# Chriz122/ultralytics_pro

Measured on AMD Instinct MI355X. Metric: images/sec (whole job = n_gpus x per-GPU bs=32) YOLOv8n 640x640 (forward + Detect decode + NMS), higher is better.
Workload: dtype bf16

## Files before the change

include/upa.h:

```cpp
#ifndef UPA_H
#define UPA_H
#include <stddef.h>
#include <stdint.h>

#ifdef __cplusplus
extern "C" {
#endif

enum { UPA_F32 = 0, UPA_BF16 = 1, UPA_U8_BGR_HWC = 2  };
enum { UPA_ACT_NONE = 0, UPA_ACT_SILU = 1, UPA_ACT_RELU = 2 };
enum { UPA_OK = 0, UPA_EINVAL = -1, UPA_EUNSUPPORTED = -2, UPA_EWORKSPACE = -3, UPA_ELAUNCH = -4 };

typedef struct upa_opts {
  uint32_t size;
  int32_t conv_big;
  int32_t conv_big_bm;
  int32_t conv_ckt;
  int32_t no_ws, no_pipe, no_1x1, no_c16, no_upcat;
  int32_t pipe_all;
  int32_t pipe_min_tiles;
  int32_t pipe_wgs, c16_wgs;
  int32_t c1_mt, c1_waves, c1_wgs;
  int32_t pair;
  int32_t pair_tile64, pair_tile32;
  int32_t no_pair_cv2;
  int32_t c2f;
  int32_t c2f16_waves;
  int32_t c2f32_th;
  int32_t no_branch_tail;
  int32_t branch_tail_bm;
  int32_t stem_wgs, stemf_wgs, stemf_waves, stem_no_mfma;
  int32_t ablate_conv, ablate_pipe, ablate_c1, ablate_stem;
  int32_t c2f64_max_px;
  int32_t conv_ws3;
  int32_t no_group;
  int32_t no_c2f32_up;
  int32_t no_xcd;
  int32_t keys_only;
  int32_t conv_p8;
  int32_t c2f_stream;
  int32_t c2f_stream_rows;
  int32_t no_stack_first;
  int32_t no_epi_stats;
  int32_t nms_stages;
  int32_t nms_first_prefix;
  int32_t detect_stream;
  int32_t detect_stream_rows;
  int32_t no_sppf_front;
  int32_t no_c2f16_down;
} upa_opts;

int upa_version(void);
const char* upa_last_error(void);
size_t upa_opts_size(void);

size_t upa_conv_packed_weight_bytes(int cout, int cin, int k, int dtype);
int upa_pack_conv_weight(const float* w_oihw, int cout, int cin, int k, int dtype, void* out);
int upa_conv2d_bias_act(const void* x, int n, int h, int w, int cin, int ldx,
                        const void* w_packed, const float* bias ,
                        void* y, int cout, int ldy,
                        const void* residual , int ldr,
                        int k, int stride, int pad, int act, int dtype, const upa_opts* opts, void* stream);
typedef struct upa_conv_problem {
  const void* x; int32_t n, h, w, cin, ldx;
  const void* w_packed; const float* bias;
  void* y; int32_t cout, ldy;
  const void* residual; int32_t ldr;
} upa_conv_problem;
int upa_conv2d_bias_act_group(const upa_conv_problem* probs, int count, int k, int stride, int pad, int act, int dtype,
                              const upa_opts* opts, void* stream);

int upa_conv2d_pool2(const void* x, int n, int h, int w, int cin, int ldx, const void* w_packed, const float* bias, void* y, int cout,
                     int ldy, int k, int stride, int pad, int act, int dtype, const upa_opts* opts, void* stream);
int upa_conv2d_stem_nchw_pool2(const void* x_nchw, int x_dtype, int n, int cin, int h, int w, const float* w_oihw, const float* bias,
                               void* y, int cout, int ldy, int k, int stride, int pad, int act, int dtype, const upa_opts* opts,
                               void* stream);

int upa_conv_variant(int n, int h, int w, int cin, int cout, int k, int stride, int pad, int dtype, const upa_opts* opts);

int upa_bottleneck_pair(const void* x, int n, int h, int w, int c, int ldx, const void* w1_packed, const float* b1,
                        const void* w2_packed, const float* b2, void* y, int ldy, int residual, int act, int dtype,
                        const upa_opts* opts, void* stream);
int upa_bottleneck_pair_e(const void* x, int n, int h, int w, int c, int cmid, int ldx, const void* w1_packed, const float* b1,
                          const void* w2_packed, const float* b2, void* y, int ldy, int residual, int act, int dtype,
                          const upa_opts* opts, void* stream);


size_t upa_stem_packed_weight_bytes(int cout, int cin, int k);
int upa_pack_stem_weight(const float* w_oihw, int cout, int cin, int k, float* out );
int upa_conv2d_stem_nchw(const void* x_nchw, int x_dtype, int n, int cin, int h, int w,
                         const float* w_oihw, const float* bias, void* y, int cout, int ldy,
                         int k, int stride, int pad, int act, int dtype, const upa_opts* opts, void* stream);

enum { UPA_STEM_SCALAR = 1, UPA_STEM_MFMA = 2, UPA_STEM_MFMA_G16 = 3, UPA_STEM_FUSED16 = 4, UPA_STEM_FUSED32 = 5 };
enum { UPA_STEM_STAGE_DMA = 0, UPA_STEM_STAGE_VGPR = 1, UPA_STEM_STAGE_U8 = 2 };
long long upa_stem_variant(int x_dtype, int n, int cin, int h, int w, int cout, int ldy, int k, int stride, int pad, int act, int dtype,
                           int pool, const upa_opts* opts, int x_align);

int upa_stem_conv_fused(const void* x, int n, int h, int w, const float* w0, const float* b0, const void* w1,
                        const float* b1, void* y, int ldy, const upa_opts* opts, void* stream);
int upa_stem_conv_fused_k(const void* x, int n, int h, int w, int k0, const float* w0, const float* b0, const void* w1,
                          const float* b1, void* y, int ldy, const upa_opts* opts, void* stream);
int upa_stem_conv_fused_c(const void* x, int n, int h, int w, int k0, int c0, const float* w0, const float* b0, const void* w1,
                          const float* b1, void* y, int ldy, const upa_opts* opts, void* stream);
int upa_stem_conv_fused_s(const void* x, int n, int h, int w, int k0, int s0, int c0, const float* w0, const float* b0,
                          const void* w1, const float* b1, void* y, int ldy, const upa_opts* opts, void* stream);

long long upa_stem_fused_variant(int n, int h, int w, int k0, int s0, int c0, int ldy, const upa_opts* opts, int x_align);

int upa_maxpool2d(const void* x, int n, int h, int w, int c, int ldx, void* y, int oh, int ow, int ldy,
                  int k, int stride, int pad, int pad_br, int dtype, void* stream);
int upa_sppf_pool3(const void* x, int n, int h, int w, int c, int ldx, void* y1, void* y2, void* y3, int ldy,
                   int dtype, void* stream);
int upa_sppf_front(const void* x, int n, int h, int w, int c1, int ldx, const void* w_packed, const float* bias, void* y, int c_, int ldy, int dtype,
                   const upa_opts* opts, void* stream);
int upa_upsample2x(const void* x, int n, int h, int w, int c, int ldx, void* y, int ldy, int dtype, void* stream);
int upa_copy_view(const void* x, int n, int h, int w, int c, int ldx, void* y, int ldy, int dtype, void* stream);
int upa_copy_to_host(const void* src_dev, void* dst_pinned, size_t bytes, void* stream);
int upa_results_to_host(const void* rows_dev, const int* counts_dev, int batch, int max_rows, int row_bytes,
                        void* rows_pinned, int* counts_pinned, void* stream);
int upa_add_view(const void* a, int lda, const void* b, int ldb, void* y, int ldy, int n, int h, int w, int c,
                 int dtype, void* stream);
int upa_nchw_to_nhwc(const float* x, int n, int c, int h, int w, void* y, int ldy, int dtype, void* stream);
int upa_nhwc_to_nchw(const void* x, int n, int h, int w, int c, int ldx, float* y, int dtype, void* stream);
int upa_letterbox_u8(const void* src, int n, int h0, int w0, long src_image_stride, int src_row_stride, void* dst, int H, int W,
                     int new_h, int new_w, int top, int left, int pad_value, void* stream);


int upa_detect_decode(const void* box, int ldb, const void* cls, int ldc, int n, int h, int w, int reg_max, int nc,
                      float stride_px, float* y, int a_total, int a0, int dtype, void* stream);
int upa_detect_tail(const void* x, int n, int h, int w, int cin, int ldx, const void* w_packed, const float* bias, int cout,
                    int kind, int nc, float stride_px, float* y, int a_total, int a0, void* raw, int ldraw,
// ... 284 lines not shown
```

ultralytics_pro_amd/_lib.py:

```python

from __future__ import annotations

import ctypes as C
import os
from pathlib import Path

import torch

UPA_F32, UPA_BF16, UPA_U8_BGR_HWC = 0, 1, 2
UPA_EINVAL = -1
UPA_EUNSUPPORTED = -2
ACT_NONE, ACT_SILU, ACT_RELU = 0, 1, 2
MASKS_PLANES, MASKS_OVERLAP = 0, 1
MASK_U8, MASK_F32, MASK_I32 = 0, 1, 2

_PKG = Path(__file__).resolve().parent
LIB_PATH = Path(os.environ.get("UPA_HIP_LIB", _PKG / "libupa_hip.so"))

_vp, _i, _f, _sz = C.c_void_p, C.c_int, C.c_float, C.c_size_t


class Opts(C.Structure):

    _fields_ = [("size", C.c_uint32), ("conv_big", _i), ("conv_big_bm", _i), ("conv_ckt", _i),
                ("no_ws", _i), ("no_pipe", _i), ("no_1x1", _i), ("no_c16", _i), ("no_upcat", _i),
                ("pipe_all", _i), ("pipe_min_tiles", _i), ("pipe_wgs", _i), ("c16_wgs", _i),
                ("c1_mt", _i), ("c1_waves", _i), ("c1_wgs", _i),
                ("pair", _i), ("pair_tile64", _i), ("pair_tile32", _i), ("no_pair_cv2", _i),
                ("c2f", _i), ("c2f16_waves", _i), ("c2f32_th", _i),
                ("no_branch_tail", _i), ("branch_tail_bm", _i),
                ("stem_wgs", _i), ("stemf_wgs", _i), ("stemf_waves", _i), ("stem_no_mfma", _i),
                ("ablate_conv", _i), ("ablate_pipe", _i), ("ablate_c1", _i), ("ablate_stem", _i), ("c2f64_max_px", _i), ("conv_ws3", _i), ("no_group", _i), ("no_c2f32_up", _i), ("no_xcd", _i), ("keys_only", _i), ("conv_p8", _i), ("c2f_stream", _i), ("c2f_stream_rows", _i), ("no_stack_first", _i), ("no_epi_stats", _i), ("nms_stages", _i), ("nms_first_prefix", _i), ("detect_stream", _i), ("detect_stream_rows", _i), ("no_sppf_front", _i), ("no_c2f16_down", _i)]

    def __init__(self, **kw):
        super().__init__()
        self.size = C.sizeof(Opts)
        for k, v in kw.items():
            if k in dict(self._fields_):
                setattr(self, k, int(v))
            else:
                raise AttributeError(f"upa_opts has no field '{k}'")

    def replace(self, **kw) -> "Opts":
        o = Opts()
        C.memmove(C.byref(o), C.byref(self), C.sizeof(Opts))
        for k, v in kw.items():
            setattr(o, k, int(v))
        return o

    _ENV = {"UPA_CONV_BIG": ("conv_big", lambda v: {0: 1, 1: 0, 2: 2}[int(v)]), "UPA_CONV_BIG_BM": ("conv_big_bm", int), "UPA_CONV_WS3": ("conv_ws3", int),
            "UPA_CONV_CKT": ("conv_ckt", int), "UPA_CONV_NO_WS": ("no_ws", lambda v: 1), "UPA_CONV_NO_PIPE": ("no_pipe", lambda v: 1),
            "UPA_CONV_NO_1X1": ("no_1x1", lambda v: 1), "UPA_CONV_NO_C16": ("no_c16", lambda v: 1), "UPA_NO_UPCAT": ("no_upcat", lambda v: 1),
            "UPA_PIPE_ALL": ("pipe_all", lambda v: 1), "UPA_PIPE_MIN_TILES": ("pipe_min_tiles", int), "UPA_PIPE_WGS": ("pipe_wgs", int),
            "UPA_C16_WGS": ("c16_wgs", int), "UPA_C1_MT": ("c1_mt", int), "UPA_C1_WAVES": ("c1_waves", int), "UPA_C1_WGS": ("c1_wgs", int),
            "UPA_NO_PAIR": ("pair", lambda v: {0: 2, 1: 1, 2: 0, 3: 3}[int(v)]), "UPA_PAIR_T64": ("pair_tile64", int),
            "UPA_PAIR_T32": ("pair_tile32", int), "UPA_NO_PAIR_CV2": ("no_pair_cv2", int), "UPA_NO_C2F": ("c2f", int),
            "UPA_C2F16_WAVES": ("c2f16_waves", int), "UPA_C2F32_TH": ("c2f32_th", int), "UPA_NO_BRANCH_TAIL": ("no_branch_tail", int),
            "UPA_BRANCH_TAIL_BM": ("branch_tail_bm", int), "UPA_STEM_WGS": ("stem_wgs", int), "UPA_STEMF_WGS": ("stemf_wgs", int),
            "UPA_STEMF_WAVES": ("stemf_waves", int), "UPA_STEM_NO_MFMA": ("stem_no_mfma", lambda v: 1),
            "UPA_CONV_ABLATE": ("ablate_conv", int), "UPA_PIPE_ABLATE": ("ablate_pipe", int), "UPA_C1_ABLATE": ("ablate_c1", int),
            "UPA_STEM_ABLATE": ("ablate_stem", int)}

    @classmethod
    def from_env(cls, env=None) -> "Opts":
        env = os.environ if env is None else env
        o = cls()
        for name, (field, conv) in cls._ENV.items():
            if name in env:
                setattr(o, field, conv(env[name]))
        return o


class BranchLevel(C.Structure):
    _fields_ = [("x", C.c_void_p), ("n", _i), ("h", _i), ("w", _i), ("c", _i), ("ldx", _i), ("w3_packed", C.c_void_p), ("b3", C.c_void_p),
                ("wt_packed", C.c_void_p), ("bt", C.c_void_p), ("stride_px", C.c_float), ("a0", _i)]


class DetectBranch(C.Structure):
    _fields_ = [("c", _i), ("reserved", _i), ("w1", C.c_void_p), ("b1", C.c_void_p), ("w2", C.c_void_p), ("b2", C.c_void_p),
                ("wt", C.c_void_p), ("bt", C.c_void_p)]


class ConvProblem(C.Structure):
    _fields_ = [("x", C.c_void_p), ("n", _i), ("h", _i), ("w", _i), ("cin", _i), ("ldx", _i), ("w_packed", C.c_void_p), ("bias", C.c_void_p),
                ("y", C.c_void_p), ("cout", _i), ("ldy", _i), ("residual", C.c_void_p), ("ldr", _i)]


_op = C.POINTER(Opts)

PROTOTYPES = {
    "upa_version": (_i, []),
    "upa_last_error": (C.c_char_p, []),
    "upa_opts_size": (_sz, []),
    "upa_conv_packed_weight_bytes": (_sz, [_i, _i, _i, _i]),
    "upa_pack_conv_weight": (_i, [_vp, _i, _i, _i, _i, _vp]),
    "upa_conv2d_bias_act": (_i, [_vp, _i, _i, _i, _i, _i, _vp, _vp, _vp, _i, _i, _vp, _i, _i, _i, _i, _i, _i, _op, _vp]),
    "upa_conv_variant": (_i, [_i, _i, _i, _i, _i, _i, _i, _i, _i, _op]),
    "upa_bottleneck_pair": (_i, [_vp, _i, _i, _i, _i, _i, _vp, _vp, _vp, _vp, _vp, _i, _i, _i, _i, _op, _vp]),
    "upa_bottleneck_pair_e": (_i, [_vp, _i, _i, _i, _i, _i, _i, _vp, _vp, _vp, _vp, _vp, _i, _i, _i, _i, _op, _vp]),
    "upa_stem_packed_weight_bytes": (_sz, [_i, _i, _i]),
    "upa_pack_stem_weight": (_i, [_vp, _i, _i, _i, _vp]),
    "upa_conv2d_stem_nchw": (_i, [_vp, _i, _i, _i, _i, _i, _vp, _vp, _vp, _i, _i, _i, _i, _i, _i, _i, _op, _vp]),
    "upa_conv2d_stem_nchw_pool2": (_i, [_vp, _i, _i, _i, _i, _i, _vp, _vp, _vp, _i, _i, _i, _i, _i, _i, _i, _op, _vp]),
    "upa_conv2d_pool2": (_i, [_vp, _i, _i, _i, _i, _i, _vp, _vp, _vp, _i, _i, _i, _i, _i, _i, _i, _op, _vp]),
    "upa_stem_conv_fused": (_i, [_vp, _i, _i, _i, _vp, _vp, _vp, _vp, _vp, _i, _op, _vp]),
    "upa_stem_conv_fused_k": (_i, [_vp, _i, _i, _i, _i, _vp, _vp, _vp, _vp, _vp, _i, _op, _vp]),
    "upa_stem_conv_fused_c": (_i, [_vp, _i, _i, _i, _i, _i, _vp, _vp, _vp, _vp, _vp, _i, _op, _vp]),
    "upa_stem_conv_fused_s": (_i, [_vp, _i, _i, _i, _i, _i, _i, _vp, _vp, _vp, _vp, _vp, _i, _op, _vp]),
    "upa_stem_variant": (C.c_longlong, [_i, _i, _i, _i, _i, _i, _i, _i, _i, _i, _i, _i, _i, _op, _i]),
    "upa_stem_fused_variant": (C.c_longlong, [_i, _i, _i, _i, _i, _i, _i, _op, _i]),
    "upa_maxpool2d": (_i, [_vp, _i, _i, _i, _i, _i, _vp, _i, _i, _i, _i, _i, _i, _i, _i, _vp]),
    "upa_sppf_pool3": (_i, [_vp, _i, _i, _i, _i, _i, _vp, _vp, _vp, _i, _i, _vp]),
    "upa_upsample2x": (_i, [_vp, _i, _i, _i, _i, _i, _vp, _i, _i, _vp]),
    "upa_copy_view": (_i, [_vp, _i, _i, _i, _i, _i, _vp, _i, _i, _vp]),
    "upa_copy_to_host": (_i, [_vp, _vp, _sz, _vp]),
# ... 181 lines not shown
```

ultralytics_pro_amd/csrc/conv_big.hip:

```cpp
#include <stdlib.h>

#include <mutex>
#include <type_traits>
#include <unordered_map>

#include "common.h"
#include "conv_pipe.h"
UPA_STAMP_DEFINE(conv_big)

template <int KS, int STRIDE, int WM, int WN, int MT, int NT, int TAIL = 0>
__device__ __forceinline__ void conv_big_body(const BigParams& p, const int bid0) {
  static_assert(WM * WN == 8, "8 waves per workgroup");
  static_assert(TAIL == 0 || TAIL == 3 || TAIL == 4 || WN == 1, "a tail needs every channel of a pixel in one wave");
  static_assert(TAIL != 1 || (NT % 2) == 0, "box branch: 64 channels");
  static_assert(TAIL != 3 || (NT % 2) == 0, "the statistics epilogue pairs n-tiles");
  static_assert(TAIL != 4 || ((NT % 2) == 0 && KS == 2 && STRIDE == 1), "the interleaving epilogue: 2 x 2 phase kernels, paired n-tiles");
  constexpr int NTB = WN * NT;
  constexpr int WBUF = 2 * NTB * 1024;
  extern __shared__ __attribute__((aligned(16))) char smem[];
  const int tid = threadIdx.x;
  const int lane = tid & 63;
  const int wave = __builtin_amdgcn_readfirstlane(tid >> 6);
  const int r = lane & 15, g = lane >> 4;
  const int wm = wave / WN, wn = wave % WN;

  const int tilesPerImg = p.tilesX * p.tilesY;
  int bid = p.no_xcd ? bid0 : upa_xcd_tile(bid0, tilesPerImg * p.N);
  const int n = bid / tilesPerImg;
  bid -= n * tilesPerImg;
  const int tyi = bid / p.tilesX;
  const int txi = bid - tyi * p.tilesX;
  const int oy0 = tyi * p.TH, ox0 = txi * p.TW;
  const int iy0 = oy0 * STRIDE - p.pad, ix0 = ox0 * STRIDE - p.pad;
  const int ntb0 = blockIdx.y * NTB;

  const int haloItems = p.IH * p.IWp * 8;
  const int haloPadded = (haloItems + 63) & ~63;
  char* hal = smem;
  char* wbuf = smem + (size_t)haloPadded * 16;

  int pl0[MT], pty[MT], ptx[MT];
#pragma unroll
  for (int i = 0; i < MT; ++i) {
    const int pp = (wm * MT + i) * 16 + r;
    int ty = (int)__umulhi((unsigned)pp, p.magicTW);
    int tx = pp - ty * p.TW;
    if (ty >= p.TH) { ty = p.TH; tx = 0; }
    pty[i] = ty;
    ptx[i] = tx;
    pl0[i] = ty < p.TH ? (ty * STRIDE) * p.IWp + tx : 0;
  }

  f32x4 acc[MT][NT];
#pragma unroll
  for (int i = 0; i < MT; ++i)
#pragma unroll
    for (int j = 0; j < NT; ++j) acc[i][j] = f32x4{0.f, 0.f, 0.f, 0.f};

  constexpr int TAPS = KS * KS;
  const int nChunks = (p.KTT + 1) >> 1;

  auto stage_halo = [&](int c) __attribute__((always_inline)) {
    const int c0 = c * 64;
    for (int base = wave * 64; base < haloPadded; base += 512) {
      const int idx = base + lane;
      const int pix = idx >> 3;
      const int slot = idx & 7;
      const int cg = slot ^ (pix & 7);
      const int py = (int)__umulhi((unsigned)pix, p.magicIW);
      const int qx = pix - py * p.IWp;
      int px = qx;
      if constexpr (STRIDE == 2) px = qx < p.HALF ? 2 * qx : 2 * (qx - p.HALF) + 1;
      const int iy = iy0 + py, ix = ix0 + px;
      const int ch = c0 + cg * 8;
      const char* src = reinterpret_cast<const char*>(g_zero16);
      if (idx < haloItems && px < p.IW && iy >= 0 && iy < p.H && ix >= 0 && ix < p.W && ch < p.Cin)
        src = p.x + ((((size_t)n * p.H + iy) * p.W + ix) * (size_t)p.ldx + ch) * 2;
      lds_dma16(src, hal + base * 16);
    }
  };
  auto stage_w = [&](int c, int tap, int b) __attribute__((always_inline)) {
#pragma unroll
    for (int f0 = 0; f0 < 2 * NTB; f0 += 8) {
      const int f = f0 + wave;
      if (f < 2 * NTB) {
        const int kt = f / NTB, j = f - kt * NTB;
        const int ktg = c * 2 + kt;
        const int nt = ntb0 + j;
        const char* src = reinterpret_cast<const char*>(g_zero16);
        if (ktg < p.KTT && nt < p.NTn) src = p.w + (((size_t)(tap * p.KTT + ktg) * p.NTn + nt) * 64 + lane) * 16;
        lds_dma16(src, wbuf + b * WBUF + f * 1024);
      }
    }
  };

  UPA_STAMP_AT(0);
  UPA_STAMP_HWID();
  stage_halo(0);
  stage_w(0, 0, 0);
  int buf = 0;
  for (int c = 0; c < nChunks; ++c) {
    int kh = 0, kw = 0;
#pragma unroll 1
    for (int tap = 0; tap < TAPS; ++tap) {
      asm volatile("s_waitcnt vmcnt(0)" ::: "memory");
      __syncthreads();
      if (c == 0) UPA_STAMP_AT(1 + tap);
      if (tap + 1 < TAPS) stage_w(c, tap + 1, buf ^ 1);
      const int tapshift = kh * p.IWp + (STRIDE == 2 ? (kw >> 1) + (kw & 1) * p.HALF : kw);
      const char* wb = wbuf + buf * WBUF + (wn * NT) * 1024 + lane * 16;
      int paddr[MT], pswz[MT];
#pragma unroll
      for (int i = 0; i < MT; ++i) {
        const int pl = pl0[i] + tapshift;
        paddr[i] = pl * 128;
        pswz[i] = pl & 7;
      }
#pragma unroll
      for (int kt = 0; kt < 2; ++kt) {
        if constexpr (TAIL == 2) {
          if (kt == 1 && c * 2 + 1 >= p.KTT) break;
        }
        if constexpr (NT <= 6) {
          u32x4 a[NT], b[MT];
#pragma unroll
          for (int j = 0; j < NT; ++j) a[j] = *reinterpret_cast<const u32x4*>(wb + (kt * NTB + j) * 1024);
#pragma unroll
          for (int i = 0; i < MT; ++i) b[i] = *reinterpret_cast<const u32x4*>(hal + paddr[i] + (((kt * 4 + g) ^ pswz[i]) << 4));
#pragma unroll
          for (int i = 0; i < MT; ++i)
#pragma unroll
            for (int j = 0; j < NT; ++j)
              acc[i][j] = __builtin_amdgcn_mfma_f32_16x16x32_bf16(*reinterpret_cast<const bf16x8*>(&a[j]),
                                                                  *reinterpret_cast<const bf16x8*>(&b[i]), acc[i][j], 0, 0, 0);
        } else {
          constexpr int GS = (NT + 1) / 2;
          u32x4 b[MT];
#pragma unroll
          for (int i = 0; i < MT; ++i) b[i] = *reinterpret_cast<const u32x4*>(hal + paddr[i] + (((kt * 4 + g) ^ pswz[i]) << 4));
#pragma unroll
          for (int j0 = 0; j0 < NT; j0 += GS) {
            u32x4 a[GS];
#pragma unroll
            for (int j = 0; j < GS; ++j)
              if (j0 + j < NT) a[j] = *reinterpret_cast<const u32x4*>(wb + (kt * NTB + j0 + j) * 1024);
#pragma unroll
            for (int i = 0; i < MT; ++i)
#pragma unroll
              for (int j = 0; j < GS; ++j)
                if (j0 + j < NT)
                  acc[i][j0 + j] = __builtin_amdgcn_mfma_f32_16x16x32_bf16(*reinterpret_cast<const bf16x8*>(&a[j]),
                                                                           *reinterpret_cast<const bf16x8*>(&b[i]), acc[i][j0 + j], 0, 0, 0);
            __builtin_amdgcn_sched_barrier(0);
          }
        }
      }
      buf ^= 1;
      if (++kw == KS) { kw = 0; ++kh; }
    }
    if (c + 1 < nChunks) {
      __syncthreads();
      stage_halo(c + 1);
      stage_w(c + 1, 0, buf);
    }
  }
  UPA_STAMP_AT(10);

  if constexpr (TAIL == 1 || TAIL == 2) {
    f32x4 bv[NT];
#pragma unroll
    for (int j = 0; j < NT; ++j) bv[j] = *reinterpret_cast<const f32x4*>(p.bias + j * 16 + g * 4);
    f32x4 acc2[MT][NT];
#pragma unroll
    for (int i = 0; i < MT; ++i)
#pragma unroll
      for (int j = 0; j < NT; ++j) acc2[i][j] = f32x4{0.f, 0.f, 0.f, 0.f};
#pragma unroll
    for (int s2 = 0; s2 < NT / 2; ++s2) {
      u32x4 hb[MT];
#pragma unroll
      for (int i = 0; i < MT; ++i) {
        float v0[4], v1[4];
#pragma unroll
        for (int q = 0; q < 4; ++q) {
          v0[q] = act_rcp<UPA_ACT_SILU>(acc[i][2 * s2][q] + bv[2 * s2][q]);
          v1[q] = act_rcp<UPA_ACT_SILU>(acc[i][2 * s2 + 1][q] + bv[2 * s2 + 1][q]);
        }
        hb[i] = u32x4{pack_bf16x2(v0[0], v0[1]), pack_bf16x2(v0[2], v0[3]), pack_bf16x2(v1[0], v1[1]), pack_bf16x2(v1[2], v1[3])};
      }
#pragma unroll
      for (int j = 0; j < NT; ++j) {
        const u32x4 a2 = *reinterpret_cast<const u32x4*>(p.tw + ((size_t)(s2 * NT + j) * 64 + lane) * 16);
#pragma unroll
        for (int i = 0; i < MT; ++i)
          acc2[i][j] = __builtin_amdgcn_mfma_f32_16x16x32_bf16(*reinterpret_cast<const bf16x8*>(&a2),
                                                               *reinterpret_cast<const bf16x8*>(&hb[i]), acc2[i][j], 0, 0, 0);
      }
    }
    if constexpr (NT & 1) {
// ... 158 lines not shown
          for (int q = 0; q < 4; ++q) {
            auto sw = __builtin_amdgcn_permlane16_swap(__float_as_uint(v0[q]), __float_as_uint(v1[q]), false, false);
            x8[q] = __uint_as_float(sw[0]);
            x8[4 + q] = __uint_as_float(sw[1]);
          }
          if (ok) {
            const u32x4 rv = *reinterpret_cast<const u32x4*>(rsrc);
#pragma unroll
            for (int q = 0; q < 4; ++q) {
              x8[2 * q] += __uint_as_float(rv[q] << 16);
              x8[2 * q + 1] += __uint_as_float(rv[q] & 0xFFFF0000u);
            }
            *reinterpret_cast<u32x4*>(dst) = u32x4{pack_bf16x2(x8[0], x8[1]), pack_bf16x2(x8[2], x8[3]),
                                                   pack_bf16x2(x8[4], x8[5]), pack_bf16x2(x8[6], x8[7])};
          }
        } else {
          auto lo = __builtin_amdgcn_permlane16_swap(pack_bf16x2(v0[0], v0[1]), pack_bf16x2(v1[0], v1[1]), false, false);
          auto hi = __builtin_amdgcn_permlane16_swap(pack_bf16x2(v0[2], v0[3]), pack_bf16x2(v1[2], v1[3]), false, false);
          if (ok) *reinterpret_cast<u32x4*>(dst) = u32x4{lo[0], hi[0], lo[1], hi[1]};
        }
      }
      if constexpr (NT & 1) {
        constexpr int j = NT - 1;
        const int cb = 16 * j + 4 * g;
        float v[4];
        const f32x4 bj = LAZY_BIAS ? bias_of(j) : biasv[LAZY_BIAS ? 0 : j];
#pragma unroll
        for (int q = 0; q < 4; ++q) v[q] = act_rcp<ACT>(acc[i][j][q] + bj[q]);
        if (pok && cw + cb < p.Cout) {
          if (p.res) {
            const u32x2 rv = *reinterpret_cast<const u32x2*>(rrow + cb * 2);
            v[0] += __uint_as_float(rv[0] << 16); v[1] += __uint_as_float(rv[0] & 0xFFFF0000u);
            v[2] += __uint_as_float(rv[1] << 16); v[3] += __uint_as_float(rv[1] & 0xFFFF0000u);
          }
          *reinterpret_cast<u32x2*>(yrow + cb * 2) = u32x2{pack_bf16x2(v[0], v[1]), pack_bf16x2(v[2], v[3])};
        }
      }
    }
  };
  if (p.act == UPA_ACT_SILU) epilogue(std::integral_constant<int, UPA_ACT_SILU>{});
  else if (p.act == UPA_ACT_RELU) epilogue(std::integral_constant<int, UPA_ACT_RELU>{});
  else epilogue(std::integral_constant<int, UPA_ACT_NONE>{});
  UPA_STAMP_AT(11);
#ifdef UPA_STAMP
  asm volatile("s_waitcnt vmcnt(0)" ::: "memory");
  UPA_STAMP_AT(12);
#endif
}

template <int KS, int STRIDE, int WM, int WN, int MT, int NT, int TAIL = 0>
__global__ __launch_bounds__(512, 4) void conv_big_kernel(const BigParams p) {
  conv_big_body<KS, STRIDE, WM, WN, MT, NT, TAIL>(p, (int)blockIdx.x);
}

template <int KS, int STRIDE, int WM, int WN, int MT, int NT, int TAIL = 0>
__global__ __launch_bounds__(512, 4) void conv_big_pair_kernel(const BigParams p0, const BigParams p1, const int split) {
  if ((int)blockIdx.x < split) conv_big_body<KS, STRIDE, WM, WN, MT, NT, TAIL>(p0, (int)blockIdx.x);
  else conv_big_body<KS, STRIDE, WM, WN, MT, NT, TAIL>(p1, (int)blockIdx.x - split);
}
template <int KS, int STRIDE, int WM, int WN, int MT, int NT, int TAIL = 0>
__global__ __launch_bounds__(512, 4) void conv_big_tri_kernel(const BigParams p0, const BigParams p1, const BigParams p2, const int s0,
                                                              const int s1) {
  if ((int)blockIdx.x < s0) conv_big_body<KS, STRIDE, WM, WN, MT, NT, TAIL>(p0, (int)blockIdx.x);
  else if ((int)blockIdx.x < s1) conv_big_body<KS, STRIDE, WM, WN, MT, NT, TAIL>(p1, (int)blockIdx.x - s0);
  else conv_big_body<KS, STRIDE, WM, WN, MT, NT, TAIL>(p2, (int)blockIdx.x - s1);
}

template <int KS_, int STRIDE_, int WM_, int WN_, int MT_, int NT_, int TAIL_>
struct BigCfg {
  static constexpr int NTB = WN_ * NT_;
  __device__ static __forceinline__ void run(const BigParams& p, int bid) { conv_big_body<KS_, STRIDE_, WM_, WN_, MT_, NT_, TAIL_>(p, bid); }
};
template <class CA, class CB>
__global__ __launch_bounds__(512, 4) void conv_big_mix_kernel(const BigParams a0, const BigParams a1, const BigParams b0, const BigParams b1,
                                                              const int s0, const int s1, const int s2) {
  const int b = (int)blockIdx.x;
  if (b < s0) CA::run(a0, b);
  else if (b < s1) CA::run(a1, b - s0);
  else if (b < s2) CB::run(b0, b - s1);
  else CB::run(b1, b - s2);
}

namespace {
void big_halo_geometry(BigParams& p, bool tight = false) {
  p.IH = (p.TH - 1) * p.stride + p.KS;
  p.IW = (p.TW - 1) * p.stride + p.KS;
  p.HALF = p.stride == 2 ? (p.IW + 1) / 2 : 0;
  const int minp = p.stride == 2 ? 2 * p.HALF : p.IW;
  p.IWp = tight ? minp : upa_lds_pick_pitch(minp, p.TW, p.TH * p.TW, p.stride);
  p.magicTW = (unsigned)((0x100000000ULL + p.TW - 1) / p.TW);
  p.magicIW = (unsigned)((0x100000000ULL + p.IWp - 1) / p.IWp);
}
size_t big_halo_bytes(const BigParams& p) { return (((size_t)p.IH * p.IWp * 8 + 63) & ~(size_t)63) * 16; }

bool big_pick_tile(BigParams& p, int bm, int ntb, size_t lds_cap) {
  struct Pick { int th, tw, tight; };
  static std::mutex mu;
  static std::unordered_map<unsigned long long, Pick> memo;
  const unsigned long long key = ((unsigned long long)p.OH << 48) ^ ((unsigned long long)p.OW << 32) ^ ((unsigned long long)bm << 20) ^
                                 ((unsigned long long)ntb << 12) ^ ((unsigned long long)(lds_cap >> 9) << 3) ^ ((unsigned long long)p.KS << 56) ^ (p.KS == 3 ? 4u : 0u) ^
                                 (p.stride == 2 ? 2u : 0u);
  {
    std::lock_guard<std::mutex> lk(mu);
    auto it = memo.find(key);
    if (it != memo.end()) {
      if (it->second.th <= 0) return false;
      p.TH = it->second.th; p.TW = it->second.tw;
      big_halo_geometry(p, it->second.tight != 0);
      return true;
    }
  }
  long best = -1;
  int bth = 0, btw = 0;
  bool btight = false;
  for (int tw = 2; tw <= 256 && tw <= ((p.OW + 1) & ~1); ++tw) {
    int th0 = bm / tw;
    if (th0 > p.OH) th0 = p.OH;
    if (th0 < 1) continue;
    const int thb = cdiv(p.OH, cdiv(p.OH, th0));
    for (int pass = 0; pass < 2; ++pass) {
      const int th = pass ? thb : th0;
      if (pass && thb == th0) break;
      for (int tight = 0; tight < 2; ++tight) {
        p.TH = th; p.TW = tw;
        big_halo_geometry(p, tight != 0);
        const size_t lds = big_halo_bytes(p) + 2 * (size_t)(2 * ntb * 1024) + 256;
        if (lds > lds_cap) continue;
        const long tiles = (long)cdiv(p.OW, tw) * cdiv(p.OH, th);
        const long cost = tiles * 65536 + (long)p.IH * p.IWp;
        if (best < 0 || cost < best) { best = cost; bth = th; btw = tw; btight = tight != 0; }
        break;
      }
    }
  }
  p.TH = bth; p.TW = btw;
  if (best >= 0) big_halo_geometry(p, btight);
  {
    std::lock_guard<std::mutex> lk(mu);
    memo[key] = Pick{best >= 0 ? bth : 0, btw, btight ? 1 : 0};
  }
  return best >= 0;
}

template <int KS, int STRIDE, int WM, int WN, int MT, int NT, int TAIL = 0>
int big_launch_inst(const BigParams& p, size_t lds, hipStream_t s) {
  constexpr int NTB = WN * NT;
  const dim3 grid((unsigned)((long)p.tilesX * p.tilesY * p.N), (unsigned)cdiv(p.NTn, NTB));
  auto kern = conv_big_kernel<KS, STRIDE, WM, WN, MT, NT, TAIL>;
  if (hipError_t e = upa_full_lds<conv_big_kernel<KS, STRIDE, WM, WN, MT, NT, TAIL>>(); e != hipSuccess) {
    upa_set_error("conv_big: cannot raise LDS limit: %s", hipGetErrorString(e));
    return UPA_ELAUNCH;
  }
  hipLaunchKernelGGL(kern, grid, dim3(512), lds, s, p);
  UPA_LAUNCH_CHECK();
  return UPA_OK;
}

template <int KS, int STRIDE, int WM, int WN, int MT, int NT, int TAIL = 0>
int big_launch_pair_inst(const BigParams& p0, const BigParams& p1, size_t lds, hipStream_t s) {
  constexpr int NTB = WN * NT;
  const long t0 = (long)p0.tilesX * p0.tilesY * p0.N, t1 = (long)p1.tilesX * p1.tilesY * p1.N;
  if (cdiv(p0.NTn, NTB) != cdiv(p1.NTn, NTB) || t0 + t1 >= (1L << 31)) return UPA_EUNSUPPORTED;
  const dim3 grid((unsigned)(t0 + t1), (unsigned)cdiv(p0.NTn, NTB));
  if (hipError_t e = upa_full_lds<conv_big_pair_kernel<KS, STRIDE, WM, WN, MT, NT, TAIL>>(); e != hipSuccess) {
    upa_set_error("conv_big: cannot raise LDS limit: %s", hipGetErrorString(e));
    return UPA_ELAUNCH;
  }
  hipLaunchKernelGGL((conv_big_pair_kernel<KS, STRIDE, WM, WN, MT, NT, TAIL>), grid, dim3(512), lds, s, p0, p1, (int)t0);
  UPA_LAUNCH_CHECK();
  return UPA_OK;
}

template <int KS, int STRIDE, int WM, int WN, int MT, int NT, int TAIL = 0>
int big_launch_tri_inst(const BigParams& p0, const BigParams& p1, const BigParams& p2, size_t lds, hipStream_t s) {
  constexpr int NTB = WN * NT;
  const long t0 = (long)p0.tilesX * p0.tilesY * p0.N, t1 = (long)p1.tilesX * p1.tilesY * p1.N, t2 = (long)p2.tilesX * p2.tilesY * p2.N;
  if (cdiv(p0.NTn, NTB) != cdiv(p1.NTn, NTB) || cdiv(p0.NTn, NTB) != cdiv(p2.NTn, NTB) || t0 + t1 + t2 >= (1L << 31)) return UPA_EUNSUPPORTED;
  const dim3 grid((unsigned)(t0 + t1 + t2), (unsigned)cdiv(p0.NTn, NTB));
  if (hipError_t e = upa_full_lds<conv_big_tri_kernel<KS, STRIDE, WM, WN, MT, NT, TAIL>>(); e != hipSuccess) {
    upa_set_error("conv_big: cannot raise LDS limit: %s", hipGetErrorString(e));
    return UPA_ELAUNCH;
  }
  hipLaunchKernelGGL((conv_big_tri_kernel<KS, STRIDE, WM, WN, MT, NT, TAIL>), grid, dim3(512), lds, s, p0, p1, p2, (int)t0, (int)(t0 + t1));
  UPA_LAUNCH_CHECK();
  return UPA_OK;
}

template <class CA, class CB>
int big_launch_mix(const BigParams* pa, int na, const BigParams* pb, int nb, size_t lds, hipStream_t s) {
  long t[4] = {0, 0, 0, 0};
  for (int i = 0; i < na; ++i) { t[i] = (long)pa[i].tilesX * pa[i].tilesY * pa[i].N; if (pa[i].NTn > CA::NTB) return UPA_EUNSUPPORTED; }
  for (int i = 0; i < nb; ++i) { t[2 + i] = (long)pb[i].tilesX * pb[i].tilesY * pb[i].N; if (pb[i].NTn > CB::NTB) return UPA_EUNSUPPORTED; }
  const long tot = t[0] + t[1] + t[2] + t[3];
  if (tot >= (1L << 31)) return UPA_EUNSUPPORTED;
  if (hipError_t e = upa_full_lds<conv_big_mix_kernel<CA, CB>>(); e != hipSuccess) {
    upa_set_error("conv_big: cannot raise LDS limit: %s", hipGetErrorString(e));
    return UPA_ELAUNCH;
  }
  hipLaunchKernelGGL((conv_big_mix_kernel<CA, CB>), dim3((unsigned)tot), dim3(512), lds, s, pa[0], pa[na > 1 ? 1 : 0], pb[0], pb[nb > 1 ? 1 : 0],
                     (int)t[0], (int)(t[0] + t[1]), (int)(t[0] + t[1] + t[2]));
  UPA_LAUNCH_CHECK();
  return UPA_OK;
}

template <int WM, int WN, int MT, int NT>
int big_launch_ks(const BigParams& p, size_t lds, hipStream_t s) {
  if (p.KS == 1) return big_launch_inst<1, 1, WM, WN, MT, NT>(p, lds, s);
  if (p.KS == 2) return big_launch_inst<2, 1, WM, WN, MT, NT>(p, lds, s);
  if (p.stride == 2) return big_launch_inst<3, 2, WM, WN, MT, NT>(p, lds, s);
  return big_launch_inst<3, 1, WM, WN, MT, NT>(p, lds, s);
}
}

extern "C" size_t upa_tail_packed_weight_bytes(int cout, int cin) {
  return (size_t)cdiv(cin, 32) * cdiv(cout, 16) * 1024;
}

static inline unsigned short big_host_bf16(float f) {
  unsigned u;
// ... 129 lines not shown
}

extern "C" int upa_detect_head_tails(const upa_branch_level* box, const upa_branch_level* cls, int count, int nc, float* y, int a_total,
                                     unsigned long long* best_keys, int dtype, const upa_opts* opts, void* stream) {
  UPA_CHECK_ARG(box && cls && count >= 1 && count <= 8, "detect_head_tails: 1..8 levels");
  BigParams pb[8], pc[8];
  int ntbb[8], bmb[8], ntbc[8], bmc[8];
  size_t ldsb[8], ldsc[8];
  for (int i = 0; i < count; ++i) {
    const upa_branch_level& b = box[i];
    const upa_branch_level& c = cls[i];
    if (const int rc = branch_tail_prepare(pb[i], ntbb[i], bmb[i], ldsb[i], b.x, b.n, b.h, b.w, b.c, b.ldx, b.w3_packed, b.b3, b.wt_packed, b.bt,
                                           1, nc, b.stride_px, y, a_total, b.a0, nullptr, dtype, opts); rc != UPA_OK)
      return rc;
    if (const int rc = branch_tail_prepare(pc[i], ntbc[i], bmc[i], ldsc[i], c.x, c.n, c.h, c.w, c.c, c.ldx, c.w3_packed, c.b3, c.wt_packed, c.bt,
                                           2, nc, c.stride_px, y, a_total, c.a0, best_keys, dtype, opts); rc != UPA_OK)
      return rc;
  }
  hipStream_t s = (hipStream_t)stream;
  const int grouping = UPA_OPT(opts, no_group);
  auto mx = [](size_t a, size_t b) { return a > b ? a : b; };
  using Box128 = BigCfg<3, 1, 8, 1, 1, 4, 1>;
  using Cls128 = BigCfg<3, 1, 8, 1, 1, 5, 2>;
  using Box256 = BigCfg<3, 1, 8, 1, 2, 4, 1>;
  using Cls256 = BigCfg<3, 1, 8, 1, 2, 5, 2>;
  for (int i = 0; i < count;) {
    if (grouping != 1 && ntbc[i] == 5) {
      if (i + 1 < count && ntbc[i + 1] == 5 && bmb[i] == 128 && bmb[i + 1] == 128 && bmc[i] == 128 && bmc[i + 1] == 128) {
        const size_t l = mx(mx(ldsb[i], ldsb[i + 1]), mx(ldsc[i], ldsc[i + 1]));
        const int rc = big_launch_mix<Cls128, Box128>(pc + i, 2, pb + i, 2, l, s);
        if (rc == UPA_OK) { i += 2; continue; }
        if (rc != UPA_EUNSUPPORTED) return rc;
      }
      if (bmb[i] == bmc[i]) {
        const size_t l = mx(ldsb[i], ldsc[i]);
        const int rc = bmb[i] == 128 ? big_launch_mix<Cls128, Box128>(pc + i, 1, pb + i, 1, l, s) : big_launch_mix<Cls256, Box256>(pc + i, 1, pb + i, 1, l, s);
        if (rc == UPA_OK) { ++i; continue; }
        if (rc != UPA_EUNSUPPORTED) return rc;
      }
    }
    if (const int rc = branch_tail_launch(pb[i], 1, ntbb[i], bmb[i], ldsb[i], s); rc != UPA_OK) return rc;
    if (const int rc = branch_tail_launch(pc[i], 2, ntbc[i], bmc[i], ldsc[i], s); rc != UPA_OK) return rc;
    ++i;
  }
  return UPA_OK;
}

bool upa_conv_big_pick_tile(BigParams& p, int bm, int ntb, size_t lds_cap) { return big_pick_tile(p, bm, ntb, lds_cap); }

bool upa_conv_big_eligible(const ConvShape& s, const upa_opts* opts) {
  const int mode = UPA_OPT(opts, conv_big);
  if (mode == 1) return false;
  const int k = s.k, stride = s.stride, cin = s.cin, cout = s.cout;
  if (s.dtype != UPA_BF16 || !((k == 1 && stride == 1) || (k == 2 && stride == 1) || (k == 3 && (stride == 1 || stride == 2))) || s.pad != k / 2) return false;
  if (cin % 8 != 0 || s.ldx % 8 != 0 || cout % 8 != 0 || s.ldy % 8 != 0 || s.ldr % 8 != 0) return false;
  if (s.act != UPA_ACT_SILU && s.act != UPA_ACT_NONE && s.act != UPA_ACT_RELU) return false;
  if (mode == 2) return cout >= 64;
  const int oh = (s.h + 2 * s.pad - k) / stride + 1, ow = (s.w + 2 * s.pad - k) / stride + 1;
  const long px = (long)s.n * oh * ow;
  if (k == 1) {
    if (cout % 128 != 0 || px < 2048) return false;
    if (cout >= 1024 && cin >= 128 && px >= 32 * 1024) return true;
    return cin >= 512 && !upa_conv1x1_eligible(s, opts);
  }
  if (cin < 64 || px < 2048) return false;
  if (cout % 128 == 0) return cin >= 128 || (px >= 8192 && (stride == 2 || px >= 200 * 1024));
  if (px < 8192) return false;
  if (cout == 80 || cout == 96) return stride == 1 && k == 3;
  if (cout == 144) return stride == 1 && k == 3;
  if (cout == 64) return stride == 1;
  return false;
}

namespace {
int big_prepare(BigParams& p, int& ntb, int& bm, size_t& lds, const upa_opts* opts, bool query_only, int force_ntb = 0) {
  p.KTT = (p.Cin + 31) / 32;
  p.NTn = (p.Cout + 15) / 16;
  ntb = p.NTn <= 4 ? 4 : (p.NTn <= 6 ? 6 : 8);
  if (p.NTn == 5 && p.KS == 3 && p.stride == 1) ntb = 5;
  if (p.NTn == 9 && p.KS == 3 && p.stride == 1) ntb = 9;
  if (force_ntb == 5 && p.NTn <= 5 && p.KS == 3 && p.stride == 1) ntb = 5;
  const long px = (long)p.N * p.OH * p.OW;
  if (ntb == 8 && p.NTn % 4 == 0 && (px + 127) / 128 * cdiv(p.NTn, 8) < upa_num_cus()) ntb = 4;
  const int cols = cdiv(p.NTn, ntb);
  bm = 256;
  if ((px + 255) / 256 * cols < upa_num_cus()) bm = 128;
  if (const int f = UPA_OPT(opts, conv_big_bm); f == 128 || f == 256 || (f == 512 && p.KS == 3 && p.stride == 1 && (ntb == 4 || ntb == 5))) bm = f;
  if (query_only) return UPA_OK;
  if (p.KS == 1) {
    p.N = 1; p.H = 1; p.W = (int)px; p.OH = 1; p.OW = (int)px;
    p.TH = 1; p.TW = bm;
    big_halo_geometry(p, true);
  } else if (!big_pick_tile(p, bm, ntb, 80 * 1024 - 512) && !big_pick_tile(p, bm, ntb, 160 * 1024)) {
    return UPA_EUNSUPPORTED;
  }
  p.tilesX = cdiv(p.OW, p.TW);
  p.tilesY = cdiv(p.OH, p.TH);
  lds = big_halo_bytes(p) + 2 * (size_t)(2 * ntb * 1024) + 256;
  if (lds > 160 * 1024) return UPA_EUNSUPPORTED;
  return UPA_OK;
}
template <int WM, int WN, int MT, int NT>
int big_launch_ks_stats(const BigParams& p, size_t lds, hipStream_t s) {
  if (p.KS == 1) return big_launch_inst<1, 1, WM, WN, MT, NT, 3>(p, lds, s);
  if (p.KS != 3) return UPA_EUNSUPPORTED;
  if (p.stride == 2) return big_launch_inst<3, 2, WM, WN, MT, NT, 3>(p, lds, s);
  return big_launch_inst<3, 1, WM, WN, MT, NT, 3>(p, lds, s);
}
int big_dispatch_stats(const BigParams& p, int ntb, int bm, size_t lds, hipStream_t s) {
  if (bm != 128 && bm != 256) return UPA_EUNSUPPORTED;
  if (ntb == 8) return bm == 256 ? big_launch_ks_stats<4, 2, 4, 4>(p, lds, s) : big_launch_ks_stats<4, 2, 2, 4>(p, lds, s);
  if (ntb == 4) return bm == 256 ? big_launch_ks_stats<8, 1, 2, 4>(p, lds, s) : big_launch_ks_stats<4, 2, 2, 2>(p, lds, s);
  return UPA_EUNSUPPORTED;
}
int big_dispatch(const BigParams& p, int ntb, int bm, size_t lds, hipStream_t s) {
  if (bm == 512) return ntb == 5 ? big_launch_inst<3, 1, 8, 1, 4, 5>(p, lds, s) : big_launch_inst<3, 1, 8, 1, 4, 4>(p, lds, s);
  if (ntb == 5) return bm == 256 ? big_launch_inst<3, 1, 8, 1, 2, 5>(p, lds, s) : big_launch_inst<3, 1, 8, 1, 1, 5>(p, lds, s);
  if (ntb == 9) return bm == 256 ? big_launch_inst<3, 1, 8, 1, 2, 9>(p, lds, s) : big_launch_inst<3, 1, 8, 1, 1, 9>(p, lds, s);
  if (ntb == 8) return bm == 256 ? big_launch_ks<4, 2, 4, 4>(p, lds, s) : big_launch_ks<4, 2, 2, 4>(p, lds, s);
  if (ntb == 6) return bm == 256 ? big_launch_ks<4, 2, 4, 3>(p, lds, s) : big_launch_ks<4, 2, 2, 3>(p, lds, s);
  return bm == 256 ? big_launch_ks<8, 1, 2, 4>(p, lds, s) : big_launch_ks<4, 2, 2, 2>(p, lds, s);
}
}

int upa_conv_big_launch(BigParams p, int query_only, int* variant, void* stream, const upa_opts* opts) {
  p.no_xcd = UPA_OPT(opts, no_xcd);
  int ntb = 0, bm = 0;
  size_t lds = 0;
  const int rc = big_prepare(p, ntb, bm, lds, opts, query_only != 0);
  if (variant) *variant = (1 << 23) | (ntb << 4) | (bm >> 7);
  if (query_only || rc != UPA_OK) return rc;
  return big_dispatch(p, ntb, bm, lds, (hipStream_t)stream);
}

int upa_conv_big_launch_interleave(BigParams p, void* stream, const upa_opts* opts) {
  p.no_xcd = UPA_OPT(opts, no_xcd);
  if (p.KS != 2 || p.stride != 1 || p.act != UPA_ACT_NONE || p.bias || p.il_c % 8 != 0 || p.Cout != 4 * p.il_c) return UPA_EUNSUPPORTED;
  int ntb = 0, bm = 0;
  size_t lds = 0;
  if (const int rc = big_prepare(p, ntb, bm, lds, opts, false); rc != UPA_OK) return rc;
  if (ntb != 8 || (bm != 128 && bm != 256)) return UPA_EUNSUPPORTED;
  hipStream_t s = (hipStream_t)stream;
  return bm == 256 ? big_launch_inst<2, 1, 4, 2, 4, 4, 4>(p, lds, s) : big_launch_inst<2, 1, 4, 2, 2, 4, 4>(p, lds, s);
}

int upa_conv_big_launch_stats(BigParams p, int* rows, long max_rows, void* stream, const upa_opts* opts) {
  p.no_xcd = UPA_OPT(opts, no_xcd);
  if (!p.stats || p.res || p.act != UPA_ACT_NONE) return UPA_EUNSUPPORTED;
  int ntb = 0, bm = 0;
  size_t lds = 0;
  if (const int rc = big_prepare(p, ntb, bm, lds, opts, false); rc != UPA_OK) return rc;
  if ((ntb != 8 && ntb != 4) || (bm != 128 && bm != 256)) return UPA_EUNSUPPORTED;
  const long nrows = (long)p.tilesX * p.tilesY * p.N;
  if (nrows > max_rows) return UPA_EUNSUPPORTED;
  p.stats_ld = p.NTn * 16;
  *rows = (int)nrows;
  return big_dispatch_stats(p, ntb, bm, lds, (hipStream_t)stream);
}

int upa_conv_big_launch_group(const BigParams* probs, int count, int* consumed, void* stream, const upa_opts* opts) {
  *consumed = 0;
  if (count < 2) return UPA_EUNSUPPORTED;
  const int grouping = UPA_OPT(opts, no_group);
  if (grouping == 1) return UPA_EUNSUPPORTED;
  if (count >= 4) {
    BigParams q[4];
    int nt4[4], bm4[4];
    size_t l4[4];
    bool ok = true;
    for (int i = 0; i < 4 && ok; ++i) {
      q[i] = probs[i];
      ok = q[i].KS == 3 && q[i].stride == 1 && big_prepare(q[i], nt4[i], bm4[i], l4[i], opts, false) == UPA_OK && bm4[i] == 128;
    }
    if (ok && nt4[0] == 4 && nt4[1] == 4 && nt4[2] == 5 && nt4[3] == 5) {
      size_t l = l4[0];
      for (int i = 1; i < 4; ++i) l = l4[i] > l ? l4[i] : l;
// ... 56 lines not shown
```

ultralytics_pro_amd/csrc/conv_pipe.h:

```cpp
#pragma once
struct ConvShape {
  int n, h, w, cin, ldx, cout, ldy, ldr, k, stride, pad, act, dtype;
};
struct PipeParams {
  const char* x;
  char* y;
  const char* res;
  const char* w;
  const float* bias;
  int N, H, W, Cin, ldx, Cout, ldy, ldr;
  int KTT, NTn, nt0;
  int tilesX, tilesY, numTiles;
  int act;
  int pool;
#ifdef UPA_ABLATE
  int ablate;
#endif
};
bool upa_conv_pipe_eligible(const ConvShape& s, const upa_opts* opts);
int upa_conv_pipe_launch(PipeParams p, int query_only, int* variant, void* stream, const upa_opts* opts);

#include "detect_epi.h"
struct C1Params {
  const char* x;
  char* y;
  const char* w;
  const float* bias;
  int P;
  int Cin, ldx, Cout, ldy;
  int KTT, NTn, groups;
  int act;
#ifdef UPA_ABLATE
  int ablate;
#endif
  int epi;
  DetectEpi de;
  float* stats;
  int stats_ld;
  const char* up;
  int upKT, up_ld, upH, upW;
  unsigned upMagicW, upMagicH;
};
bool upa_conv1x1_eligible(const ConvShape& s, const upa_opts* opts);
int upa_conv1x1_launch(C1Params p, int n_pixels, int query_only, int* variant, void* stream, const upa_opts* opts);
int upa_conv1x1_launch_stats(C1Params p, int n_pixels, int* rows, long max_rows, void* stream, const upa_opts* opts);

struct BigParams {
  const char* x;
  char* y;
  const char* res;
  const char* w;
  const float* bias;
  int N, H, W, Cin, ldx, OH, OW, Cout, ldy, ldr;
  int KS, stride, pad;
  int TH, TW, tilesX, tilesY, IH, IW;
  int IWp;
  int HALF;
  int KTT, NTn;
  int act;
  unsigned magicTW, magicIW;
  int no_xcd;
  const char* tw;
  const float* tb;
  DetectEpi de;
  float* stats;
  int stats_ld;
  int il_h, il_w, il_c;
};
bool upa_conv_big_eligible(const ConvShape& s, const upa_opts* opts);
int upa_conv_big_launch(BigParams p, int query_only, int* variant, void* stream, const upa_opts* opts);
int upa_conv_big_launch_stats(BigParams p, int* rows, long max_rows, void* stream, const upa_opts* opts);
int upa_conv_big_launch_interleave(BigParams p, void* stream, const upa_opts* opts);
int upa_conv_big_launch_group(const BigParams* probs, int count, int* consumed, void* stream, const upa_opts* opts);

bool upa_conv_big_pick_tile(BigParams& p, int bm, int ntb, size_t lds_cap);

bool upa_conv_p8_eligible(const ConvShape& s, const upa_opts* opts);
int upa_conv_p8_launch(BigParams p, int query_only, int* variant, void* stream, const upa_opts* opts);

bool upa_conv_ws3_eligible(const ConvShape& s, const upa_opts* opts);
int upa_conv_ws3_launch(BigParams p, int query_only, int* variant, void* stream, const upa_opts* opts);
int upa_conv_ws3_launch_stats(BigParams p, int* rows, long max_rows, void* stream, const upa_opts* opts);

struct PairParams {
  const char* x;
  char* y;
  const char* w1;
  const char* w2;
  const float* b1;
  const float* b2;
  int N, H, W, OH, OW, ldx, ldy;
  int TH, TW, tilesX, tilesY;
  int IWp, MWp;
  unsigned magicIW, magicMW, magicTW;
  const char* y0;
  const char* wc_std;
  const char* wc_b;
  const float* bc;
  char* out; int ldout;
};
```

Measured before the change: 61600.

## Add keyed LDS swizzle for stride-2 halo to cut bank conflicts

For stride-2 3x3 convolutions, the halo is now staged at the tight pitch, with an XOR swizzle key derived from the row parity and a displacement chosen by a bank-conflict cost model. This replaces the padded pitch, so the LDS footprint shrinks while bank conflicts stay low. An optional mode also widens the n-tile block to 8 when enough workgroups remain. The risks are extra index arithmetic in staging and loads, and possible mismatches if the key math is wrong.

Measured after the change: 61390. No clear change (-0.3%).

```diff
diff --git a/include/upa.h b/include/upa.h
--- a/include/upa.h
+++ b/include/upa.h
@@ -48,6 +48,7 @@
   int32_t detect_stream_rows;
   int32_t no_sppf_front;
   int32_t no_c2f16_down;
+  int32_t conv_big_s2_layout;
 } upa_opts;
 
 int upa_version(void);
diff --git a/ultralytics_pro_amd/_lib.py b/ultralytics_pro_amd/_lib.py
--- a/ultralytics_pro_amd/_lib.py
+++ b/ultralytics_pro_amd/_lib.py
@@ -30,7 +30,7 @@
                 ("c2f", _i), ("c2f16_waves", _i), ("c2f32_th", _i),
                 ("no_branch_tail", _i), ("branch_tail_bm", _i),
                 ("stem_wgs", _i), ("stemf_wgs", _i), ("stemf_waves", _i), ("stem_no_mfma", _i),
-                ("ablate_conv", _i), ("ablate_pipe", _i), ("ablate_c1", _i), ("ablate_stem", _i), ("c2f64_max_px", _i), ("conv_ws3", _i), ("no_group", _i), ("no_c2f32_up", _i), ("no_xcd", _i), ("keys_only", _i), ("conv_p8", _i), ("c2f_stream", _i), ("c2f_stream_rows", _i), ("no_stack_first", _i), ("no_epi_stats", _i), ("nms_stages", _i), ("nms_first_prefix", _i), ("detect_stream", _i), ("detect_stream_rows", _i), ("no_sppf_front", _i), ("no_c2f16_down", _i)]
+                ("ablate_conv", _i), ("ablate_pipe", _i), ("ablate_c1", _i), ("ablate_stem", _i), ("c2f64_max_px", _i), ("conv_ws3", _i), ("no_group", _i), ("no_c2f32_up", _i), ("no_xcd", _i), ("keys_only", _i), ("conv_p8", _i), ("c2f_stream", _i), ("c2f_stream_rows", _i), ("no_stack_first", _i), ("no_epi_stats", _i), ("nms_stages", _i), ("nms_first_prefix", _i), ("detect_stream", _i), ("detect_stream_rows", _i), ("no_sppf_front", _i), ("no_c2f16_down", _i), ("conv_big_s2_layout", _i)]
 
     def __init__(self, **kw):
         super().__init__()
diff --git a/ultralytics_pro_amd/csrc/conv_big.hip b/ultralytics_pro_amd/csrc/conv_big.hip
--- a/ultralytics_pro_amd/csrc/conv_big.hip
+++ b/ultralytics_pro_amd/csrc/conv_big.hip
@@ -40,6 +40,9 @@
   char* wbuf = smem + (size_t)haloPadded * 16;
 
   int pl0[MT], pty[MT], ptx[MT];
+  [[maybe_unused]] int swd = 0, swe = 0;
+  if constexpr (STRIDE == 2) { swd = p.SWK & 7; swe = p.SWK >> 4; }
+  [[maybe_unused]] int pk0[MT];
 #pragma unroll
   for (int i = 0; i < MT; ++i) {
     const int pp = (wm * MT + i) * 16 + r;
@@ -49,6 +52,7 @@
     pty[i] = ty;
     ptx[i] = tx;
     pl0[i] = ty < p.TH ? (ty * STRIDE) * p.IWp + tx : 0;
+    if constexpr (STRIDE == 2) pk0[i] = ty < p.TH ? ty * swd + tx : 0;
   }
 
   f32x4 acc[MT][NT];
@@ -66,9 +70,10 @@
       const int idx = base + lane;
       const int pix = idx >> 3;
       const int slot = idx & 7;
-      const int cg = slot ^ (pix & 7);
+      int cg = slot ^ (pix & 7);
       const int py = (int)__umulhi((unsigned)pix, p.magicIW);
       const int qx = pix - py * p.IWp;
+      if constexpr (STRIDE == 2) cg = slot ^ ((qx + (py >> 1) * swd + (py & 1) * swe) & 7);
       int px = qx;
       if constexpr (STRIDE == 2) px = qx < p.HALF ? 2 * qx : 2 * (qx - p.HALF) + 1;
       const int iy = iy0 + py, ix = ix0 + px;
@@ -108,6 +113,8 @@
       if (c == 0) UPA_STAMP_AT(1 + tap);
       if (tap + 1 < TAPS) stage_w(c, tap + 1, buf ^ 1);
       const int tapshift = kh * p.IWp + (STRIDE == 2 ? (kw >> 1) + (kw & 1) * p.HALF : kw);
+      [[maybe_unused]] int tapkey = 0;
+      if constexpr (STRIDE == 2) tapkey = (kw >> 1) + (kw & 1) * p.HALF + (kh >> 1) * swd + (kh & 1) * swe;
       const char* wb = wbuf + buf * WBUF + (wn * NT) * 1024 + lane * 16;
       int paddr[MT], pswz[MT];
 #pragma unroll
@@ -115,6 +122,7 @@
         const int pl = pl0[i] + tapshift;
         paddr[i] = pl * 128;
         pswz[i] = pl & 7;
+        if constexpr (STRIDE == 2) pswz[i] = (pk0[i] + tapkey) & 7;
       }
 #pragma unroll
       for (int kt = 0; kt < 2; ++kt) {
@@ -439,31 +447,40 @@
 }
 
 namespace {
-void big_halo_geometry(BigParams& p, bool tight = false) {
+void big_halo_geometry(BigParams& p, bool tight = false, bool keyed = false) {
   p.IH = (p.TH - 1) * p.stride + p.KS;
   p.IW = (p.TW - 1) * p.stride + p.KS;
   p.HALF = p.stride == 2 ? (p.IW + 1) / 2 : 0;
   const int minp = p.stride == 2 ? 2 * p.HALF : p.IW;
-  p.IWp = tight ? minp : upa_lds_pick_pitch(minp, p.TW, p.TH * p.TW, p.stride);
+  if (p.stride == 2 && keyed) {
+    p.IWp = minp;
+    int best = 0, best_cost = 1 << 30;
+    for (int d = 0; d < 8; d += 2)
+      if (const int c = upa_lds_conflict_cycles(p.TW, p.TH * p.TW, d); c < best_cost) { best_cost = c; best = d; }
+    p.SWK = best;
+  } else {
+    p.IWp = tight ? minp : upa_lds_pick_pitch(minp, p.TW, p.TH * p.TW, p.stride);
+    p.SWK = ((2 * p.IWp) & 7) | (p.IWp & 7) << 4;
+  }
   p.magicTW = (unsigned)((0x100000000ULL + p.TW - 1) / p.TW);
   p.magicIW = (unsigned)((0x100000000ULL + p.IWp - 1) / p.IWp);
 }
 size_t big_halo_bytes(const BigParams& p) { return (((size_t)p.IH * p.IWp * 8 + 63) & ~(size_t)63) * 16; }
 
-bool big_pick_tile(BigParams& p, int bm, int ntb, size_t lds_cap) {
+bool big_pick_tile(BigParams& p, int bm, int ntb, size_t lds_cap, bool keyed = false) {
   struct Pick { int th, tw, tight; };
   static std::mutex mu;
   static std::unordered_map<unsigned long long, Pick> memo;
   const unsigned long long key = ((unsigned long long)p.OH << 48) ^ ((unsigned long long)p.OW << 32) ^ ((unsigned long long)bm << 20) ^
                                  ((unsigned long long)ntb << 12) ^ ((unsigned long long)(lds_cap >> 9) << 3) ^ ((unsigned long long)p.KS << 56) ^ (p.KS == 3 ? 4u : 0u) ^
-                                 (p.stride == 2 ? 2u : 0u);
+                                 (p.stride == 2 ? 2u : 0u) ^ (p.stride == 2 && keyed ? 1u : 0u);
   {
     std::lock_guard<std::mutex> lk(mu);
     auto it = memo.find(key);
     if (it != memo.end()) {
       if (it->second.th <= 0) return false;
       p.TH = it->second.th; p.TW = it->second.tw;
-      big_halo_geometry(p, it->second.tight != 0);
+      big_halo_geometry(p, it->second.tight != 0, keyed);
       return true;
     }
   }
@@ -480,7 +497,7 @@
       if (pass && thb == th0) break;
       for (int tight = 0; tight < 2; ++tight) {
         p.TH = th; p.TW = tw;
-        big_halo_geometry(p, tight != 0);
+        big_halo_geometry(p, tight != 0, keyed);
         const size_t lds = big_halo_bytes(p) + 2 * (size_t)(2 * ntb * 1024) + 256;
         if (lds > lds_cap) continue;
         const long tiles = (long)cdiv(p.OW, tw) * cdiv(p.OH, th);
@@ -491,7 +508,7 @@
     }
   }
   p.TH = bth; p.TW = btw;
-  if (best >= 0) big_halo_geometry(p, btight);
+  if (best >= 0) big_halo_geometry(p, btight, keyed);
   {
     std::lock_guard<std::mutex> lk(mu);
     memo[key] = Pick{best >= 0 ? bth : 0, btw, btight ? 1 : 0};
@@ -787,6 +804,16 @@
   if (force_ntb == 5 && p.NTn <= 5 && p.KS == 3 && p.stride == 1) ntb = 5;
   const long px = (long)p.N * p.OH * p.OW;
   if (ntb == 8 && p.NTn % 4 == 0 && (px + 127) / 128 * cdiv(p.NTn, 8) < upa_num_cus()) ntb = 4;
+  const bool s2 = p.KS == 3 && p.stride == 2;
+  const int s2_mode = s2 ? UPA_OPT(opts, conv_big_s2_layout) : 1;
+  const bool keyed = s2 && s2_mode != 1;
+  if (s2 && (s2_mode == 2 || s2_mode == 3) && ntb == 4 && p.NTn % 8 == 0) {
+    BigParams q = p;
+    if (big_pick_tile(q, 128, 8, 80 * 1024 - 512, keyed) || big_pick_tile(q, 128, 8, 160 * 1024, keyed)) {
+      const long wgs = (long)cdiv(q.OW, q.TW) * cdiv(q.OH, q.TH) * q.N * (q.NTn / 8);
+      if (s2_mode == 3 || wgs >= upa_num_cus()) ntb = 8;
+    }
+  }
   const int cols = cdiv(p.NTn, ntb);
   bm = 256;
   if ((px + 255) / 256 * cols < upa_num_cus()) bm = 128;
@@ -796,7 +823,7 @@
     p.N = 1; p.H = 1; p.W = (int)px; p.OH = 1; p.OW = (int)px;
     p.TH = 1; p.TW = bm;
     big_halo_geometry(p, true);
-  } else if (!big_pick_tile(p, bm, ntb, 80 * 1024 - 512) && !big_pick_tile(p, bm, ntb, 160 * 1024)) {
+  } else if (!big_pick_tile(p, bm, ntb, 80 * 1024 - 512, keyed) && !big_pick_tile(p, bm, ntb, 160 * 1024, keyed)) {
     return UPA_EUNSUPPORTED;
   }
   p.tilesX = cdiv(p.OW, p.TW);
diff --git a/ultralytics_pro_amd/csrc/conv_pipe.h b/ultralytics_pro_amd/csrc/conv_pipe.h
--- a/ultralytics_pro_amd/csrc/conv_pipe.h
+++ b/ultralytics_pro_amd/csrc/conv_pipe.h
@@ -60,6 +60,7 @@
   int act;
   unsigned magicTW, magicIW;
   int no_xcd;
+  int SWK;
   const char* tw;
   const float* tb;
   DetectEpi de;
```
